# Academich/translation-transformer

Measured on AMD Instinct MI355X. Metric: reactions/sec (SMILES decoded), greedy speculative, higher is better.
Workload: dtype f32

## Files before the change

include/ttx.h:

```cpp
#ifndef TTX_H
#define TTX_H

#include <stdint.h>

#ifdef __cplusplus
extern "C" {
#endif

#define TTX_ABI_VERSION 4

typedef enum ttx_status {
  TTX_OK = 0,
  TTX_ERR_INVALID = -1,
  TTX_ERR_HIP = -2,
  TTX_ERR_NO_DEVICE = -3,
  TTX_ERR_REFERENCE = -4,
  TTX_ERR_NOMEM = -5,
  TTX_ERR_ROW_REPLAY = -6,
  TTX_ERR_MAX_STEPS = -7
} ttx_status;

typedef struct ttx_config {
  int32_t vocab_size;
  int32_t src_vocab_size;
// ... 230 lines not shown
                           float* d_kcache, float* d_vcache, int64_t cache_layer_stride, int64_t cache_seq_stride, int N, int D, int d,
                           int B, int Ld, const int32_t* d_pos2, const float* d_qkv_probe, int64_t probe_layer_stride, void* stream);

int ttx_debug_probe_split(ttx_session* s, const int32_t* d_act_idx, const int32_t* d_pred_probe, const int32_t* d_drafts, int B, int N,
                          int D, int n_active, int32_t* d_act2, int32_t* d_pos2, int32_t* result, void* stream);

int ttx_debug_merge_pred(ttx_session* s, const int32_t* d_pos2, const int32_t* d_pred_probe, const int32_t* d_pred2, int32_t* d_pred,
                         int B, int N, int D, int n_active, void* stream);

int ttx_debug_probe_split_select(ttx_session* s, const int32_t* d_act_idx, const int32_t* d_pred_probe, const int32_t* d_drafts, int B,
                                 int N, int D, int n_active, int32_t* d_act2, int32_t* d_pos2, int32_t* d_draft_mask, int32_t* d_row_base,
                                 int32_t* d_row_map, int32_t* result, void* stream);
int ttx_debug_merge_pred_select(ttx_session* s, const int32_t* d_pos2, const int32_t* d_pred_probe, const int32_t* d_pred2,
                                int32_t* d_pred, int B, int N, int D, int n_active, const int32_t* d_row_base,
                                const int32_t* d_draft_mask, void* stream);
int ttx_debug_kvcopy_select(ttx_session* s, const int32_t* d_rec, int n_copy, const float* d_qkv, int64_t qkv_layer_stride,
                            float* d_kcache, float* d_vcache, int64_t cache_layer_stride, int64_t cache_seq_stride, int N, int D, int d,
                            int B, int Ld, const int32_t* d_pos2, const float* d_qkv_probe, int64_t probe_layer_stride,
                            const int32_t* d_row_base, const int32_t* d_draft_mask, void* stream);
int ttx_debug_embed_select(ttx_session* s, const float* d_table, int V, const float* d_pe, int pe_rows, int d, float* d_x,
                           const int32_t* d_act_idx, const int32_t* d_front, const int32_t* d_gen, int gen_ld, const int32_t* d_drafts,
                           int B, int N, int D, int n_active, const int32_t* d_row_map, int m_rows, void* stream);
int ttx_debug_attn_select(ttx_session* s, const float* d_q, int ldq, const float* d_k, const float* d_v, int ldkv, float* d_out, int H,
                          float scale, int Lk, const int32_t* d_tok, int pad, const uint8_t* d_key_pad, const int32_t* d_act_idx,
                          const int32_t* d_front, const int32_t* d_src_of, const int32_t* d_src_len, const float* d_kcache,
                          const float* d_vcache, int64_t cache_seq_stride, const int32_t* d_cache_slot, int gen_ld, int N, int D, int mode,
                          int groups, int n_active, int max_keys, int kernel, int32_t* kernel_id, const int32_t* d_row_base,
                          const int32_t* d_draft_mask, void* stream);

int ttx_pool_last_counters(ttx_session* s, int64_t* counters);

int ttx_attn_staged_key_limit(int head_dim, int q_per_group);

#ifdef __cplusplus
}
#endif
#endif
```

translation-transformer_amd/_native.py:

```python
from __future__ import annotations

import ctypes as C
import os
import subprocess
from pathlib import Path

PKG_DIR = Path(__file__).resolve().parent
CSRC = PKG_DIR / "csrc"
INCLUDE = PKG_DIR.parent / "include"
LIB_PATH = PKG_DIR / "libttx_hip.so"
UNITS = [CSRC / "ttx_api.hip", CSRC / "ttx_gemm.hip", CSRC / "ttx_attn.hip"]
HEADERS = [CSRC / "ttx_internal.h", CSRC / "ttx_common.hip.h", CSRC / "ttx_loop_kernels.hip.h", CSRC / "ttx_metrics.hip.h",
           CSRC / "ttx_score.hip.h", CSRC / "ttx_select.h", CSRC / "ttx_tokenizer.h", INCLUDE / "ttx.h"]
SOURCES = UNITS + HEADERS
OBJ_DIR = CSRC / "build"

TTX_OK, TTX_ERR_INVALID, TTX_ERR_HIP, TTX_ERR_NO_DEVICE, TTX_ERR_REFERENCE, TTX_ERR_NOMEM = 0, -1, -2, -3, -4, -5
TTX_ERR_ROW_REPLAY = -6
TTX_ERR_MAX_STEPS = -7
TTX_ACT_NONE, TTX_ACT_RELU, TTX_ACT_GELU = 0, 1, 2
ACTIVATIONS = {"relu": TTX_ACT_RELU, "gelu": TTX_ACT_GELU}


def activation_code(activation: str) -> int:
# ... 117 lines not shown
    "ttx_tokenizer_encode": (C.c_int, [_VP, C.c_char_p, _VP, _I]),
    "ttx_tokenizer_encode_batch": (C.c_int, [_VP, C.POINTER(C.c_char_p), _I, _VP, _I]),
    "ttx_tokenizer_decode": (C.c_int, [_VP, _VP, _I, _VP, _I]),
    "ttx_debug_step_snapshot": (C.c_int, [_VP, C.POINTER(C.c_int32), _VP, _VP, _VP, _VP]),
    "ttx_debug_gemm_bench": (C.c_int, [_VP, _I, _I, _I, _I, _I, _I, C.POINTER(C.c_double), C.POINTER(C.c_double)]),
    "ttx_debug_gemm": (C.c_int, [_VP, _VP, _I, _VP, _I, _VP, _VP, _I, _VP, _I, _I, _I, _I, _I, C.c_int64, _I, _I,
                                 C.POINTER(C.c_int32), _VP]),
    "ttx_debug_gemm_act": (C.c_int, [_VP, _VP, _I, _VP, _I, _VP, _VP, _I, _VP, _I, _I, _I, _I, _I, C.c_int64, _I, _I,
                                     C.POINTER(C.c_int32), _VP]),
    "ttx_debug_finish_ln": (C.c_int, [_VP, _VP, _I, C.c_int64, _VP, _VP, _VP, _VP, _VP, _VP, _VP, _VP, _VP, _I, _I, C.c_float, _VP]),
    "ttx_debug_attn": (C.c_int, [_VP, _VP, _I, _VP, _VP, _I, _VP, _I, C.c_float, _I, _I, _VP, _I, _VP, _VP, _VP, _VP, _VP, _VP, _VP, _VP,
                                 C.c_int64, _VP, _I, _I, _I, _I, _I, _I, _I, _I, C.POINTER(C.c_int32), _VP]),
    "ttx_debug_attn_hd": (C.c_int, [_VP, _VP, _I, _VP, _VP, _I, _VP, _I, _I, C.c_float, _I, _I, _VP, _I, _VP, _VP, _VP, _VP, _VP, _VP, _VP,
                                    _VP, C.c_int64, _VP, _I, _I, _I, _I, _I, _I, _I, _I, C.POINTER(C.c_int32), _VP]),
    "ttx_debug_attn_as": (C.c_int, [_VP, _VP, _I, _VP, _VP, _I, _VP, _I, _I, C.c_float, _I, _I, _VP, _I, _VP, _VP, _VP, _VP, _VP, _VP, _VP,
                                    _VP, C.c_int64, _VP, _I, _I, _I, _I, _I, _I, _I, _I, C.POINTER(C.c_int32), _I, _I, _VP]),
    "ttx_debug_argmax": (C.c_int, [_VP, _VP, _I, _VP, _VP, _I, _VP]),
    "ttx_debug_embed": (C.c_int, [_VP, _VP, _I, _VP, _I, _I, _VP, _VP, _I, _I, _VP, _VP, _VP, _I, _VP, _I, _I, _I, _I, _I, _VP]),
    "ttx_debug_accept": (C.c_int, [_VP, C.POINTER(DebugAcceptArgs), C.POINTER(C.c_int64), _VP]),
    "ttx_debug_kvcopy": (C.c_int, [_VP, _VP, _I, _VP, C.c_int64, _VP, _VP, C.c_int64, C.c_int64, _I, _I, _I, _I, _I, _VP]),
    "ttx_debug_kvcopy_split": (C.c_int, [_VP, _VP, _I, _VP, C.c_int64, _VP, _VP, C.c_int64, C.c_int64, _I, _I, _I, _I, _I, _VP, _VP,
                                         C.c_int64, _VP]),
    "ttx_debug_probe_split": (C.c_int, [_VP, _VP, _VP, _VP, _I, _I, _I, _I, _VP, _VP, C.POINTER(C.c_int32), _VP]),
    "ttx_debug_merge_pred": (C.c_int, [_VP, _VP, _VP, _VP, _VP, _I, _I, _I, _I, _VP]),
    "ttx_debug_probe_split_select": (C.c_int, [_VP, _VP, _VP, _VP, _I, _I, _I, _I, _VP, _VP, _VP, _VP, _VP, C.POINTER(C.c_int32), _VP]),
    "ttx_debug_merge_pred_select": (C.c_int, [_VP, _VP, _VP, _VP, _VP, _I, _I, _I, _I, _VP, _VP, _VP]),
    "ttx_debug_kvcopy_select": (C.c_int, [_VP, _VP, _I, _VP, C.c_int64, _VP, _VP, C.c_int64, C.c_int64, _I, _I, _I, _I, _I, _VP, _VP,
                                          C.c_int64, _VP, _VP, _VP]),
    "ttx_debug_embed_select": (C.c_int, [_VP, _VP, _I, _VP, _I, _I, _VP, _VP, _VP, _VP, _I, _VP, _I, _I, _I, _I, _VP, _I, _VP]),
    "ttx_debug_attn_select": (C.c_int, [_VP, _VP, _I, _VP, _VP, _I, _VP, _I, C.c_float, _I, _VP, _I, _VP, _VP, _VP, _VP, _VP, _VP, _VP,
                                        C.c_int64, _VP, _I, _I, _I, _I, _I, _I, _I, _I, C.POINTER(C.c_int32), _VP, _VP, _VP]),
    "ttx_pool_last_counters": (C.c_int, [_VP, C.POINTER(C.c_int64)]),
    "ttx_attn_staged_key_limit": (C.c_int, [_I, _I]),
    "ttx_last_kernel_profile": (C.c_int, [_VP, C.POINTER(C.c_double), C.POINTER(C.c_int64), C.POINTER(C.c_double)]),
}

_lib = None


def hipcc_path() -> str:
    for cand in (os.environ.get("HIPCC"), "/opt/rocm/bin/hipcc", "hipcc"):
        if cand and (os.path.isabs(cand) and os.path.exists(cand) or not os.path.isabs(cand)):
            return cand
    return "hipcc"


def needs_build() -> bool:
    if not LIB_PATH.exists():
        return True
    t = LIB_PATH.stat().st_mtime
    return any(src.stat().st_mtime > t for src in SOURCES)


def build(force: bool = False, verbose: bool = False) -> Path:
    if not force and not needs_build():
        return LIB_PATH
    OBJ_DIR.mkdir(exist_ok=True)
    flags = ["--offload-arch=gfx950", "-O3", "-std=c++17", "-fPIC", f"-I{INCLUDE}"] + os.environ.get("TTX_HIPCC_FLAGS", "").split()
    newest_header = max(h.stat().st_mtime for h in HEADERS)
    jobs, objs = [], []
    for unit in UNITS:
        obj = OBJ_DIR / (unit.stem + ".o")
        objs.append(str(obj))
        if not force and obj.exists() and obj.stat().st_mtime > max(unit.stat().st_mtime, newest_header) \
                and not os.environ.get("TTX_HIPCC_FLAGS"):
            continue
# ... 41 lines not shown
```

translation-transformer_amd/csrc/ttx_api.hip:

```cpp
#include "ttx_internal.h"
#include "ttx_loop_kernels.hip.h"
#include "ttx_metrics.hip.h"
#include "ttx_score.hip.h"
#include "ttx_tokenizer.h"

#include <algorithm>
#include <chrono>
#include <cmath>
#include <cstdio>
#include <cstdlib>
#include <cstring>
#include <mutex>
#include <type_traits>

using namespace ttx;

static thread_local std::string g_err;

int ttx::fail(int code, const std::string& msg) {
  g_err = msg;
  return code;
}

static void layout_add(ttx_model* m, const std::string& name, size_t numel, size_t* off_out) {
// ... 249 lines not shown
    if (hipMemset(b.p, 0xFF, want) != hipSuccess) return fail(TTX_ERR_HIP, "hipMemset (poison) failed");
    (void)hipDeviceSynchronize();
  }
  return TTX_OK;
}

extern "C" int ttx_session_create(ttx_model* m, ttx_session** out) {
  if (!m || !out) return fail(TTX_ERR_INVALID, "null argument");
  HIP_TRY(hipSetDevice(m->device));
  ttx_session* s = new ttx_session();
  s->m = m;
  if (hipHostMalloc((void**)&s->host_info, sizeof(HostInfo), hipHostMallocMapped) != hipSuccess ||
      hipHostMalloc((void**)&s->probe_info, sizeof(ProbeInfo), hipHostMallocMapped) != hipSuccess ||
      hipHostMalloc((void**)&s->host_state, sizeof(DecState), hipHostMallocDefault) != hipSuccess) {
    if (s->host_info) (void)hipHostFree(s->host_info);
    if (s->probe_info) (void)hipHostFree(s->probe_info);
    if (s->host_state) (void)hipHostFree(s->host_state);
    delete s;
    return fail(TTX_ERR_NOMEM, "hipHostMalloc failed");
  }
  std::memset(s->host_info, 0, sizeof(HostInfo));
  std::memset(s->probe_info, 0, sizeof(ProbeInfo));
  HIP_TRY(hipEventCreate(&s->ev_a));
  HIP_TRY(hipEventCreate(&s->ev_b));
  HIP_TRY(hipEventCreate(&s->ev_c));
  HIP_TRY(hipEventCreateWithFlags(&s->ev_done, hipEventDisableTiming));
  s->use_graphs = getenv("TTX_NO_GRAPH") == nullptr;
  const char* pf = getenv("TTX_PROFILE_GEMM");
  s->profile = pf && pf[0] == '1';
  if (const char* e = getenv("TTX_SMALL_ROWS")) s->small_rows = std::max(0, atoi(e));
  if (const char* e = getenv("TTX_FFN2_SLAB_ROWS")) s->ffn2_slab_rows = std::max(0, atoi(e));
  if (const char* e = getenv("TTX_QKV_SMALL_ROWS")) s->qkv_small_rows = std::max(0, atoi(e));
  if (const char* e = getenv("TTX_ATTN_FALLBACK")) s->attn_fallback = atoi(e) != 0;
  s->host_timing = getenv("TTX_HOST_TIMING") != nullptr;
  m->n_sessions++;
  *out = s;
  return TTX_OK;
}

extern "C" void ttx_session_destroy(ttx_session* s) {
  if (!s) return;
  if (s->host_timing && s->host_launches)
    fprintf(stderr, "[ttx host timing] hipGraphLaunch: %lld launches, %.1f us each\n", s->host_launches,
            s->host_launch_us / (double)s->host_launches);
  if (s->host_timing && s->host_captures)
    fprintf(stderr, "[ttx host timing] graphs captured: %lld, %.1f us each\n", s->host_captures,
            s->host_capture_us / (double)s->host_captures);
  if (s->dead) {
    delete s;
    return;
  }
  release_retired();
  (void)hipDeviceSynchronize();
  for (Buf* b : s->all)
    if (b->p) (void)hipFree(b->p);
  if (s->host_info) (void)hipHostFree(s->host_info);
  if (s->probe_info) (void)hipHostFree(s->probe_info);
  if (s->beam_host) (void)hipHostFree(s->beam_host);
  if (s->bp_host) (void)hipHostFree(s->bp_host);
  s->drop_graphs();
  release_own_stream(s);
  if (s->ev_done) (void)hipEventDestroy(s->ev_done);
  if (s->host_state) (void)hipHostFree(s->host_state);
  for (auto& e : s->ev_pool) { (void)hipEventDestroy(e.first); (void)hipEventDestroy(e.second); }
  if (s->ev_a) (void)hipEventDestroy(s->ev_a);
  if (s->ev_b) (void)hipEventDestroy(s->ev_b);
// ... 2782 lines not shown
  MergePredArgs mp{};
  mp.st = dst; mp.pos2 = d_pos2; mp.pred_probe = d_pred_probe; mp.pred2 = d_pred2; mp.pred = d_pred; mp.RPS = step_rps(N, D);
  mp.row_base = d_row_base; mp.draft_mask = d_draft_mask; mp.D = D;
  hipLaunchKernelGGL(k_merge_pred, dim3(cdiv(B * mp.RPS, 256)), dim3(256), 0, st, mp);
  hipError_t err = hipGetLastError();
  const hipError_t esync = hipStreamSynchronize(st);
  (void)hipFree(dst);
  HIP_TRY(err);
  HIP_TRY(esync);
  return TTX_OK;
}

extern "C" int ttx_debug_merge_pred(ttx_session* s, const int32_t* d_pos2, const int32_t* d_pred_probe, const int32_t* d_pred2,
                                    int32_t* d_pred, int B, int N, int D, int n_active, void* stream) {
  return merge_pred_debug(s, d_pos2, d_pred_probe, d_pred2, d_pred, B, N, D, n_active, nullptr, nullptr, stream);
}

extern "C" int ttx_debug_merge_pred_select(ttx_session* s, const int32_t* d_pos2, const int32_t* d_pred_probe, const int32_t* d_pred2,
                                           int32_t* d_pred, int B, int N, int D, int n_active, const int32_t* d_row_base,
                                           const int32_t* d_draft_mask, void* stream) {
  if ((d_row_base != nullptr) != (d_draft_mask != nullptr))
    return fail(TTX_ERR_INVALID, "ttx_debug_merge_pred_select: row_base and draft_mask come together");
  return merge_pred_debug(s, d_pos2, d_pred_probe, d_pred2, d_pred, B, N, D, n_active, d_row_base, d_draft_mask, stream);
}

extern "C" int ttx_pool_last_counters(ttx_session* s, int64_t* counters) {
  if (!s || !counters) return fail(TTX_ERR_INVALID, "null argument to ttx_pool_last_counters");
  for (int i = 0; i < 7; ++i) counters[i] = s->pool_counters[i];
  return TTX_OK;
}

extern "C" int ttx_attn_staged_key_limit(int head_dim, int q_per_group) { return attn_staged_key_limit(head_dim, q_per_group); }

extern "C" int ttx_last_kernel_profile(ttx_session* s, double* gemm_ms, int64_t* gemm_launches, double* empty_pair_ms) {
  if (!s) return fail(TTX_ERR_INVALID, "null session");
  if (gemm_ms) *gemm_ms = s->prof_ms;
  if (gemm_launches) *gemm_launches = s->prof_launches;
  s->prof_ms = 0;
  s->prof_launches = 0;
  if (empty_pair_ms) *empty_pair_ms = s->prof_empty_pair_ms < 0 ? 0.0 : s->prof_empty_pair_ms;
  return TTX_OK;
}
```

translation-transformer_amd/csrc/ttx_attn.hip:

```cpp
#include "ttx_internal.h"

#include <algorithm>

namespace ttx {

constexpr int ATT_MAXQ = 16;
constexpr int ATT_SQ = ATT_MAXQ + 1;

__host__ __device__ inline size_t attn_lds_bytes(int max_keys, int dh) {
  return sizeof(float) * ((size_t)ATT_MAXQ * dh + (size_t)max_keys * ATT_SQ + ATT_MAXQ);
}

template <int DH, class KeyPtr, class Vis>
__device__ __forceinline__ void attn_core(const float* __restrict__ q, int ldq, int nq, int nk, KeyPtr keyptr, Vis vis,
                                          float* __restrict__ out, int ldo, float scale, float* lds) {
  const int lane = threadIdx.x & 63;
  float* Qs = lds;
  float* S = lds + ATT_MAXQ * DH;
  float* inv = S + (size_t)nk * ATT_SQ;

  for (int e = lane * 4; e < nq * DH; e += 256) {
    const int i = e / DH, c = e % DH;
    *reinterpret_cast<float4*>(&Qs[i * DH + c]) = *reinterpret_cast<const float4*>(q + (size_t)i * ldq + c);
  }
// ... 824 lines not shown
    float mx, rs, fa, fb;
    f32x16 oi;
    a3_tile_partial<MODE>(a, cu, cur, cq, it * 32, r, h, magic, mx, rs, oi);
    a3_fold(m, l, mx, rs, fa, fb);
#pragma unroll
    for (int i = 0; i < 16; ++i) o[i] = __fmaf_rn(o[i], fa, __fmul_rn(oi[i], fb));
    cur = nxt;
    if (!last) {
      ++it;
      continue;
    }
    if (SEL ? cq.orow >= 0 : r < cu.nq) {
      const float inv = l > 0.f ? 1.0f / l : 0.f;
      float* op = cu.out + (size_t)(SEL ? cq.orow : r) * a.d + 4 * h;
#pragma unroll
      for (int v = 0; v < 4; ++v) {
        f32x4 w = {o[4 * v] * inv, o[4 * v + 1] * inv, o[4 * v + 2] * inv, o[4 * v + 3] * inv};
        *reinterpret_cast<f32x4*>(op + 8 * v) = w;
      }
    }
    if (!more) break;
    cu = nu;
    cq = nq;
    un += W;
    nu = unit(min(un, n_units - 1));
    it = 0;
    m = -INFINITY;
    l = 0.f;
#pragma unroll
    for (int i = 0; i < 16; ++i) o[i] = 0.f;
  }
}

static constexpr size_t kAttn2LdsLimit = 150 * 1024;

template <int MODE, int DH>
static int launch_attn_mode(ttx_session* s, hipStream_t st, const AttnArgs& a, int groups, int H, int q_per_group, int max_keys, int N, int D1) {
  if (groups <= 0 || q_per_group <= 0) return TTX_OK;
  constexpr bool step = (MODE == ATT_STEP_SELF || MODE == ATT_STEP_CROSS);
  const int D = D1 - 1;
  const int force = s->attn_force;
  const bool want3 = force ? (force == AK_ATTN3 || force == AK_ATTN3S) : !s->attn_fallback;
  const bool want2 = force ? force == AK_ATTN2 : !s->attn_fallback;
  if ((force == AK_ATTN3 || force == AK_ATTN3S) && !(step && H % 4 == 0 && DH == ATT_DH))
    return fail(TTX_ERR_INVALID, "k_attn3 / k_attn3s serve the step modes at head dimension 32 with a head count that is a multiple of 4");
  const bool sel = a.row_base != nullptr;
  if (sel && !(step && DH == ATT_DH && H % 4 == 0 && want3 && a.draft_mask && N <= 32 && D >= 1))
    return fail(TTX_ERR_INVALID, "draft select runs on k_attn3 / k_attn3s only: a step launch at head dimension 32, a head count that is a "
                                 "multiple of 4, 1 <= N <= 32 and D >= 1");
  if constexpr (step && DH == ATT_DH) {
    if (H % 4 == 0 && want3) {
      const int qtiles = cdiv(q_per_group, A3_QT);
      const int keys3 = (MODE == ATT_STEP_SELF) ? max_keys + 1 + N * std::max(D, 0) : max_keys;
      const size_t lds3 = sizeof(float) * (size_t)A3_PART * cdiv(keys3, 32);
      bool split = s->attn_split != 0 && (s->attn_split > 0 || (long long)groups * H * qtiles < TTX_A3_SPLIT_BELOW) && lds3 <= 64 * 1024;
      if (force == AK_ATTN3 && lds3 > 64 * 1024) return fail(TTX_ERR_INVALID, "k_attn3: the parked tile partials exceed 64 KB of LDS");
      if (force) split = (force == AK_ATTN3);
      s->last_attn_kernel = split ? AK_ATTN3 : AK_ATTN3S;
      if (split) {
        if (sel) hipLaunchKernelGGL((k_attn3<MODE, true>), dim3(groups, H, qtiles), dim3(256), lds3, st, a);
        else hipLaunchKernelGGL((k_attn3<MODE, false>), dim3(groups, H, qtiles), dim3(256), lds3, st, a);
      } else {
        const long long units = (long long)groups * H * qtiles;
        const int wgs = (int)std::min<long long>((units + 3) / 4, (long long)TTX_A3S_WGS_PER_CU * s->m->n_cu);
        if (sel) hipLaunchKernelGGL((k_attn3s<MODE, true>), dim3(wgs), dim3(256), 0, st, a, H, qtiles);
        else hipLaunchKernelGGL((k_attn3s<MODE, false>), dim3(wgs), dim3(256), 0, st, a, H, qtiles);
      }
      HIP_TRY(hipGetLastError());
      return TTX_OK;
    }
  }
  const int draft_keys = (D > 0) ? (std::min(N, (A2_QT + D - 2) / D + 1)) * D : 0;
  const int keys2 = (MODE == ATT_STEP_SELF) ? max_keys + 1 + draft_keys : max_keys;
  const size_t lds2 = attn2_lds_bytes(keys2, a2_qcap(q_per_group), DH);
  if (force == AK_ATTN2 && !(lds2 <= kAttn2LdsLimit && attn2_fits(keys2, DH)))
    return fail(TTX_ERR_INVALID, "k_attn2: more keys than its register and LDS images hold");
  bool fits2 = lds2 <= kAttn2LdsLimit && attn2_fits(keys2, DH);
  if (step && s->attn_sel_N > 0) {
    const int cN = s->attn_sel_N, cD = s->attn_sel_D;
    const int c_draft = (cD > 0) ? (std::min(cN, (A2_QT + cD - 2) / cD + 1)) * cD : 0;
    const int c_keys2 = (MODE == ATT_STEP_SELF) ? max_keys + 1 + c_draft : max_keys;
    fits2 = fits2 && attn2_lds_bytes(c_keys2, a2_qcap(step_rps(cN, cD)), DH) <= kAttn2LdsLimit && attn2_fits(c_keys2, DH);
  }
  if (fits2 && want2) {
    s->last_attn_kernel = AK_ATTN2;
    const int tiles = cdiv(q_per_group, A2_QT);
    bool& attr_set = s->attr_attn2[DH == ATT_DH ? 0 : 1][MODE];
    if (lds2 > 64 * 1024 && !attr_set) {
      HIP_TRY(hipFuncSetAttribute(reinterpret_cast<const void*>(&k_attn2<MODE, DH>), hipFuncAttributeMaxDynamicSharedMemorySize,
                                  (int)kAttn2LdsLimit));
      attr_set = true;
    }
    hipLaunchKernelGGL((k_attn2<MODE, DH>), dim3(groups, H, tiles), dim3(256), lds2, st, a);
    HIP_TRY(hipGetLastError());
    return TTX_OK;
  }
  const int keys1 = (MODE == ATT_STEP_SELF) ? max_keys + q_per_group : max_keys;
  const size_t lds = attn_lds_bytes(keys1, DH);
  if (lds > kAttn2LdsLimit) return fail(TTX_ERR_INVALID, "sequence too long for the attention kernels' LDS score buffer");
  if (lds > 64 * 1024)
    HIP_TRY(hipFuncSetAttribute(reinterpret_cast<const void*>(&k_attn<MODE, DH>), hipFuncAttributeMaxDynamicSharedMemorySize, (int)lds));
  s->last_attn_kernel = AK_ATTN;
  hipLaunchKernelGGL((k_attn<MODE, DH>), dim3(groups, H, cdiv(q_per_group, ATT_MAXQ)), dim3(64), lds, st, a);
  HIP_TRY(hipGetLastError());
  return TTX_OK;
}

template <int DH>
static int launch_attn_dh(int mode, ttx_session* s, hipStream_t st, const AttnArgs& a, int groups, int H, int q_per_group, int max_keys,
                          int N, int D1) {
  switch (mode) {
    case ATT_ENC: return launch_attn_mode<ATT_ENC, DH>(s, st, a, groups, H, q_per_group, max_keys, N, D1);
    case ATT_FULL_SELF: return launch_attn_mode<ATT_FULL_SELF, DH>(s, st, a, groups, H, q_per_group, max_keys, N, D1);
    case ATT_FULL_CROSS: return launch_attn_mode<ATT_FULL_CROSS, DH>(s, st, a, groups, H, q_per_group, max_keys, N, D1);
    case ATT_STEP_SELF: return launch_attn_mode<ATT_STEP_SELF, DH>(s, st, a, groups, H, q_per_group, max_keys, N, D1);
    case ATT_STEP_CROSS: return launch_attn_mode<ATT_STEP_CROSS, DH>(s, st, a, groups, H, q_per_group, max_keys, N, D1);
  }
  return fail(TTX_ERR_INVALID, "unknown attention mode");
}

int launch_attn(int mode, ttx_session* s, hipStream_t st, const AttnArgs& a, int groups, int H, int q_per_group, int max_keys,
                int N, int D1) {
  if (H > 0 && a.d == H * 32) return launch_attn_dh<32>(mode, s, st, a, groups, H, q_per_group, max_keys, N, D1);
  if (H > 0 && a.d == H * 64) return launch_attn_dh<64>(mode, s, st, a, groups, H, q_per_group, max_keys, N, D1);
  return fail(TTX_ERR_INVALID, "attention kernels exist for head dimensions 32 and 64");
}

int attn_staged_key_limit(int head_dim, int q_per_group) {
  if ((head_dim != 32 && head_dim != 64) || q_per_group <= 0) return 0;
  int keys = 32 * a2_vsteps(head_dim);
  while (keys > 0 && attn2_lds_bytes(keys, a2_qcap(q_per_group), head_dim) > kAttn2LdsLimit) keys -= 32;
  return keys;
}

static bool attn_aligned16(const void* p) { return (reinterpret_cast<uintptr_t>(p) & 15) == 0; }

int attn_debug(ttx_session* s, const AttnArgs& in, int H, int head_dim, int mode, int groups, int n_active, int max_keys, int kernel,
               int32_t* kernel_id, hipStream_t st) {
  if (!s) return fail(TTX_ERR_INVALID, "null session");
  if (head_dim != 32 && head_dim != 64) return fail(TTX_ERR_INVALID, "ttx_debug_attn_hd: head_dim is 32 or 64");
  if (mode < ATT_ENC || mode > ATT_STEP_CROSS || kernel < 0 || kernel > AK_ATTN3S)
    return fail(TTX_ERR_INVALID, "ttx_debug_attn: mode is 0..4, kernel 0..4");
  if (H <= 0 || groups <= 0 || max_keys <= 0) return fail(TTX_ERR_INVALID, "ttx_debug_attn: H, groups and max_keys must be positive");
  const bool step = (mode == ATT_STEP_SELF || mode == ATT_STEP_CROSS);
  const bool cross = (mode == ATT_FULL_CROSS || mode == ATT_STEP_CROSS);
  AttnArgs a = in;
  a.d = H * head_dim;
  if (!a.q || !a.k || !a.v || !a.out) return fail(TTX_ERR_INVALID, "ttx_debug_attn: q, k, v and out are required");
  if (cross ? !a.key_pad : !a.tok) return fail(TTX_ERR_INVALID, "ttx_debug_attn: self modes need tok, cross modes key_pad");
  if (step && !a.act_idx) return fail(TTX_ERR_INVALID, "ttx_debug_attn: the step modes need act_idx");
  if (mode == ATT_STEP_SELF && (!a.front || !a.kcache || !a.vcache))
    return fail(TTX_ERR_INVALID, "ttx_debug_attn: STEP_SELF needs front, kcache and vcache");
  if ((a.ldq & 3) || (a.ldkv & 3) || a.ldq < a.d || a.ldkv < a.d)
    return fail(TTX_ERR_INVALID, "ttx_debug_attn: ldq and ldkv must be multiples of 4 that cover d = head_dim * H");
  for (const void* p : {(const void*)a.q, (const void*)a.k, (const void*)a.v, (const void*)a.out, (const void*)a.kcache, (const void*)a.vcache})
    if (!attn_aligned16(p)) return fail(TTX_ERR_INVALID, "ttx_debug_attn: float operands must be 16-byte aligned");
  int q_per_group = a.L;
  if (step) {
    if (a.N < 1 || a.D < 0) return fail(TTX_ERR_INVALID, "ttx_debug_attn: step modes need N >= 1 and D >= 0");
    if (n_active < 0 || n_active > groups) return fail(TTX_ERR_INVALID, "ttx_debug_attn: n_active must lie in [0, groups]");
    if (mode == ATT_STEP_SELF && (a.gen_ld <= 0 || a.cache_seq_stride <= 0 || (a.cache_seq_stride & 3)))
      return fail(TTX_ERR_INVALID, "ttx_debug_attn: STEP_SELF needs gen_ld > 0 and a cache_seq_stride that is a positive multiple of 4");
    q_per_group = step_rps(a.N, a.D);
  } else if (a.L <= 0 || (mode != ATT_FULL_CROSS && max_keys < a.L)) {
    return fail(TTX_ERR_INVALID, "ttx_debug_attn: L must be positive and max_keys cover it");
  }
  if (cross && (a.Lk <= 0 || max_keys < a.Lk)) return fail(TTX_ERR_INVALID, "ttx_debug_attn: Lk must be positive and max_keys cover it");
  HIP_TRY(hipSetDevice(s->m->device));
  DecState* dst = nullptr;
  if (step) {
    HIP_TRY(hipMalloc((void**)&dst, sizeof(DecState)));
    hipError_t e = hipMemsetAsync(dst, 0, sizeof(DecState), st);
    if (e == hipSuccess) e = hipMemsetD32Async(reinterpret_cast<hipDeviceptr_t>(&dst->n_active), n_active, 1, st);
    if (e != hipSuccess) { (void)hipFree(dst); HIP_TRY(e); }
    a.st = dst;
// ... 17 lines not shown
```

translation-transformer_amd/csrc/ttx_internal.h:

```cpp
#pragma once
#include "ttx.h"
#include "ttx_common.hip.h"

#include <map>
#include <set>
#include <string>
#include <utility>
#include <vector>

namespace ttx {
struct BeamHost;
struct BeamPoolHost;
}

struct LayerW {
  size_t sa_in_w, sa_in_b, sa_out_w, sa_out_b;
  size_t ca_in_w, ca_in_b, ca_out_w, ca_out_b;
  size_t l1_w, l1_b, l2_w, l2_b;
  size_t n1_w, n1_b, n2_w, n2_b, n3_w, n3_b;
};

struct ttx_model {
  ttx_config cfg;
  int device;
  int activation = TTX_ACT_RELU;
  int n_sessions = 0;

  int n_cu = 256;
  float* blob = nullptr;
  size_t blob_floats = 0;
  std::map<std::string, std::pair<size_t, size_t>> index;
  std::vector<LayerW> enc, dec;
  size_t src_emb, tgt_emb, enc_norm_w, enc_norm_b, dec_norm_w, dec_norm_b, cls_w, cls_b, pe;
  size_t cross_kv_w, cross_kv_b;
  const float* p(size_t off) const { return blob + off; }
};

struct Buf {
  void* p = nullptr;
  size_t cap = 0;
  uint64_t* owner_gen = nullptr;
  template <typename T> T* as() const { return reinterpret_cast<T*>(p); }
};

enum GemmVariant { GV_BIG = 0, GV_SMALL = 1, GV_BIG_FFN2_SLABS = 2, GV_MID = 3 };

enum GemmKernelId { GK_GEMM3 = 1, GK_GEMM_TN = 2, GK_GEMM24_4 = 3, GK_GEMM24_0 = 4, GK_GEMM2_1 = 5, GK_GEMM2_2 = 6, GK_GEMM2_4 = 7,
                    GK_GEMM2_0 = 8, GK_BODY_128x64 = 16 };

enum AttnKernelId { AK_ATTN = 1, AK_ATTN2 = 2, AK_ATTN3 = 3, AK_ATTN3S = 4 };

enum GraphSite { GS_STEP_SPECULATIVE = 0, GS_STEP_GREEDY = 1, GS_STEP_ROW_RULE = 2, GS_STEP_POOL = 3, GS_BEAM_ITER = 4, GS_BEAM_POOL_ITER = 5 };
typedef std::vector<int> GraphKey;

struct GraphCache {
  std::map<GraphKey, hipGraphExec_t> map;
  std::set<GraphKey> warmed;
  size_t limit;
  explicit GraphCache(size_t limit_) : limit(limit_) {}
  void clear() {
    for (auto& kv : map) (void)hipGraphExecDestroy(kv.second);
    map.clear(); warmed.clear();
  }
};

#define TTX_SESSION_BUFS(X)                                                                                                      \
                                                                      \
  X(x) X(x1) X(x2) X(xf) X(ao) X(q2) X(hbuf) X(slab) X(qkv) X(logits) X(ckv)                                                      \
                                                                                                                    \
  X(tok_src) X(src_valid) X(memory) X(memkv)                                                                                     \
                                                                                                               \
  X(tok_tgt) X(mem_pad_tmp)                                                                                                      \
   \
  X(ev_logits) X(ev_pred) X(ev_nll)                                                                                              \
   \
                                                                                                      \
  X(sc_src_of)                                                                                                                   \
                                                                                                                       \
  X(drafts) X(gen) X(front) X(act_idx) X(rec) X(pred) X(state) X(kcache) X(vcache) X(src32) X(outbuf) X(haspad) X(traj)           \
  X(fin_step)                                                                                                                    \
                                                                                            \
  X(rstep) X(row_of) X(src_len) X(new_slot) X(pool_io) X(memkv_new) X(valid_new) X(drafts_new)                                    \
       \
// ... 17 lines not shown
#ifndef TTX_BIG_MIN_TILES
#define TTX_BIG_MIN_TILES 400
#endif
struct ttx_session {
  ttx_model* m;
  std::vector<Buf*> all;
  TTX_SESSION_BUFS(TTX_DECLARE_BUF)
  Buf tk[2], tv[2];
  int snap_B = 0, snap_rps = 0, snap_gen_ld = 0, snap_step = 0;
  ttx::ProbeInfo* probe_info = nullptr;
  long long pool_counters[7] = {};
  ttx::BeamHost* beam_host = nullptr;
  ttx::BeamPoolHost* bp_host = nullptr;
  ttx::HostInfo* host_info = nullptr;
  hipStream_t own_stream = nullptr;
  uint64_t alloc_generation = 0;
  uint64_t graphs_generation = 0;
  bool dead = false;
  bool use_graphs = true;
  GraphCache step_graphs{512};
  GraphCache iter_graphs{256};
  hipEvent_t ev_done = nullptr;
  void drop_graphs() { step_graphs.clear(); iter_graphs.clear(); }
  void graphs_current() { if (graphs_generation != alloc_generation) { drop_graphs(); graphs_generation = alloc_generation; } }
  ttx::DecState* host_state = nullptr;
  bool attr_attn2[2][8] = {};
  bool attr_select = false, attr_step = false, attr_topk = false, attr_pool_select = false;
  int qkv_small_rows = 800;
  int small_rows = 2000;
  int ffn2_slab_rows = 5600;
  int big_min_tiles = TTX_BIG_MIN_TILES;
  int last_gemm_kernel = 0, last_gemm_big_min_tiles = 0;
  int attn_split = -1;
  bool attn_fallback = false;
  int attn_force = 0;
  int attn_sel_N = 0, attn_sel_D = 0;
  int last_attn_kernel = 0;
  bool profile = false;
  std::vector<std::pair<hipEvent_t, hipEvent_t>> ev_pool;
  size_t ev_used = 0;
  double prof_ms = 0;
  double prof_empty_pair_ms = -1;
  long long prof_launches = 0;
  bool host_timing = false;
  double host_launch_us = 0;
  long long host_captures = 0;
  double host_capture_us = 0;
  long long host_launches = 0;
  hipEvent_t ev_a = nullptr, ev_b = nullptr, ev_c = nullptr;
  ttx_session() {
    TTX_SESSION_BUFS(TTX_REGISTER_BUF)
    for (Buf* b : {&tk[0], &tk[1], &tv[0], &tv[1]}) all.push_back(b);
    for (Buf* b : all) b->owner_gen = &alloc_generation;
  }
};

namespace ttx {

int fail(int code, const std::string& msg);

#define HIP_TRY(expr)                                                                                  \
  do {                                                                                                 \
    hipError_t _e = (expr);                                                                            \
    if (_e != hipSuccess)                                                                              \
      return ttx::fail(TTX_ERR_HIP, std::string(#expr) + ": " + hipGetErrorString(_e) + " (" __FILE__ ":" + \
                                        std::to_string(__LINE__) + ")");                               \
  } while (0)

#define TTX_TRY(expr)        \
  do {                       \
// ... 33 lines not shown
```

translation-transformer_amd/model.py:

```python
from __future__ import annotations

import ctypes as C
import os
import math
from typing import NamedTuple

import numpy as np
import torch

from . import _native as N


def reference_pe_table(emb: int, max_len: int = 5000) -> torch.Tensor:
    pe = torch.zeros(max_len, emb)
    position = torch.arange(0, max_len, dtype=torch.float).unsqueeze(1)
    div_term = torch.exp(torch.arange(0, emb, 2).float() * (-math.log(10000.0) / emb))
    pe[:, 0::2] = torch.sin(position * div_term)
    pe[:, 1::2] = torch.cos(position * div_term)
    return torch.vstack((torch.zeros(1, emb), pe)).contiguous()


def _strip(state: dict) -> dict:
    if any(k.startswith("model.") for k in state):
        return {k[len("model."):]: v for k, v in state.items() if k.startswith("model.")}
# ... 258 lines not shown
                            row_base: torch.Tensor | None, draft_mask: torch.Tensor | None) -> None:
        assert kcache.stride() == vcache.stride()
        N.check(self._lib.ttx_debug_kvcopy_select(self._session, rec.data_ptr(), int(n_copy), qkv.data_ptr(), int(qkv.stride(0)),
                                                  kcache.data_ptr(), vcache.data_ptr(), int(kcache.stride(0)), int(kcache.stride(1)),
                                                  int(n), int(d), int(width), int(B), int(qkv.shape[0]), self._ptr(pos2),
                                                  self._ptr(qkv_probe), 0 if qkv_probe is None else int(qkv_probe.stride(0)),
                                                  self._ptr(row_base), self._ptr(draft_mask), self._stream()))

    def debug_embed_select(self, table: torch.Tensor, pe: torch.Tensor, x: torch.Tensor, act_idx: torch.Tensor, front: torch.Tensor,
                           gen: torch.Tensor, drafts: torch.Tensor, B: int, n: int, d: int, n_active: int,
                           row_map: torch.Tensor | None, m_rows: int) -> None:
        N.check(self._lib.ttx_debug_embed_select(self._session, table.data_ptr(), int(table.shape[0]), pe.data_ptr(), int(pe.shape[0]),
                                                 int(table.shape[1]), x.data_ptr(), act_idx.data_ptr(), front.data_ptr(),
                                                 gen.data_ptr(), int(gen.stride(0)), drafts.data_ptr(), int(B), int(n), int(d),
                                                 int(n_active), self._ptr(row_map), int(m_rows), self._stream()))

    def debug_attn_select(self, mode: int, q: torch.Tensor, k: torch.Tensor, v: torch.Tensor, out: torch.Tensor, heads: int,
                          scale: float, groups: int, max_keys: int, row_base: torch.Tensor | None, draft_mask: torch.Tensor | None,
                          Lk: int = 0, tok: torch.Tensor | None = None, pad: int = 0, key_pad: torch.Tensor | None = None,
                          act_idx: torch.Tensor | None = None, front: torch.Tensor | None = None, src_of: torch.Tensor | None = None,
                          src_len: torch.Tensor | None = None, kcache: torch.Tensor | None = None, vcache: torch.Tensor | None = None,
                          cache_seq_stride: int = 0, cache_slot: torch.Tensor | None = None, gen_ld: int = 0, n: int = 1, d: int = 0,
                          n_active: int = 0, kernel: int = 0, **unused) -> int:
        kid = C.c_int32(0)
        assert k.stride(0) == v.stride(0)
        N.check(self._lib.ttx_debug_attn_select(self._session, q.data_ptr(), q.stride(0), k.data_ptr(), v.data_ptr(), k.stride(0),
                                                out.data_ptr(), int(heads), float(scale), int(Lk), self._ptr(tok), int(pad),
                                                self._ptr(key_pad), self._ptr(act_idx), self._ptr(front), self._ptr(src_of),
                                                self._ptr(src_len), self._ptr(kcache), self._ptr(vcache), int(cache_seq_stride),
                                                self._ptr(cache_slot), int(gen_ld), int(n), int(d), int(mode), int(groups),
                                                int(n_active), int(max_keys), int(kernel), C.byref(kid), self._ptr(row_base),
                                                self._ptr(draft_mask), self._stream()))
        return int(kid.value)

    POOL_COUNTERS = ("steps", "split_steps", "slot_steps_probed", "slots_matched", "drafts_matched", "rows_executed", "draft_select")

    def pool_last_counters(self, session=None) -> dict:
        words = (C.c_int64 * 7)()
        N.check(self._lib.ttx_pool_last_counters(self._session if session is None else session, words))
        return dict(zip(self.POOL_COUNTERS, (int(v) for v in words)))

    @staticmethod
    def attn_staged_key_limit(head_dim: int, q_per_group: int) -> int:
        return int(N.lib().ttx_attn_staged_key_limit(int(head_dim), int(q_per_group)))

    def close(self) -> None:
        if getattr(self, "_score_session", None):
            self._lib.ttx_session_destroy(self._score_session)
            self._score_session = None
        for extra in getattr(self, "_pool", [])[1:]:
            self._lib.ttx_session_destroy(extra)
        self._pool = None
        if getattr(self, "_session", None):
            self._lib.ttx_session_destroy(self._session)
            self._session = None
        if getattr(self, "_model", None):
            self._lib.ttx_model_destroy(self._model)
            self._model = None

    def __del__(self):
        try:
            self.close()
        except Exception:
            pass

    def _tokens(self, t: torch.Tensor) -> torch.Tensor:
# ... 181 lines not shown
```

Baseline: 21430.

## Add single-row step attention kernel with two heads per 64-thread block

Adds k_attn1, a step-attention kernel for one query row at head dimension 32. Each 64-lane block handles two heads, keeps K tiles staged in LDS and prefetches the next tile while an online softmax accumulates. By default it replaces k_attn3s for unsplit, non-select launches with one query per group, aiming to cut launch width and LDS overhead for tiny decode steps. It also adds a per-session bitmask of attention kernels used, plus a debug accessor. The risk is lower occupancy and serial key tiles on long keys, and speculative launches may not reach this path at all.

```diff
diff --git a/include/ttx.h b/include/ttx.h
--- a/include/ttx.h
+++ b/include/ttx.h
@@ -286,6 +286,8 @@
 
 int ttx_attn_staged_key_limit(int head_dim, int q_per_group);
 
+int ttx_debug_attn_kernels_seen(ttx_session* s);
+
 #ifdef __cplusplus
 }
 #endif
diff --git a/translation-transformer_amd/_native.py b/translation-transformer_amd/_native.py
--- a/translation-transformer_amd/_native.py
+++ b/translation-transformer_amd/_native.py
@@ -173,6 +173,7 @@
                                         C.c_int64, _VP, _I, _I, _I, _I, _I, _I, _I, _I, C.POINTER(C.c_int32), _VP, _VP, _VP]),
     "ttx_pool_last_counters": (C.c_int, [_VP, C.POINTER(C.c_int64)]),
     "ttx_attn_staged_key_limit": (C.c_int, [_I, _I]),
+    "ttx_debug_attn_kernels_seen": (C.c_int, [_VP]),
     "ttx_last_kernel_profile": (C.c_int, [_VP, C.POINTER(C.c_double), C.POINTER(C.c_int64), C.POINTER(C.c_double)]),
 }
 
diff --git a/translation-transformer_amd/csrc/ttx_api.hip b/translation-transformer_amd/csrc/ttx_api.hip
--- a/translation-transformer_amd/csrc/ttx_api.hip
+++ b/translation-transformer_amd/csrc/ttx_api.hip
@@ -305,6 +305,7 @@
   if (const char* e = getenv("TTX_FFN2_SLAB_ROWS")) s->ffn2_slab_rows = std::max(0, atoi(e));
   if (const char* e = getenv("TTX_QKV_SMALL_ROWS")) s->qkv_small_rows = std::max(0, atoi(e));
   if (const char* e = getenv("TTX_ATTN_FALLBACK")) s->attn_fallback = atoi(e) != 0;
+  if (const char* e = getenv("TTX_ATTN_ROW")) s->attn_row = atoi(e) != 0 ? 1 : 0;
   s->host_timing = getenv("TTX_HOST_TIMING") != nullptr;
   m->n_sessions++;
   *out = s;
@@ -3153,6 +3154,11 @@
 
 extern "C" int ttx_attn_staged_key_limit(int head_dim, int q_per_group) { return attn_staged_key_limit(head_dim, q_per_group); }
 
+extern "C" int ttx_debug_attn_kernels_seen(ttx_session* s) {
+  if (!s) return fail(TTX_ERR_INVALID, "null session");
+  return (int)s->attn_kernels_seen;
+}
+
 extern "C" int ttx_last_kernel_profile(ttx_session* s, double* gemm_ms, int64_t* gemm_launches, double* empty_pair_ms) {
   if (!s) return fail(TTX_ERR_INVALID, "null session");
   if (gemm_ms) *gemm_ms = s->prof_ms;
diff --git a/translation-transformer_amd/csrc/ttx_attn.hip b/translation-transformer_amd/csrc/ttx_attn.hip
--- a/translation-transformer_amd/csrc/ttx_attn.hip
+++ b/translation-transformer_amd/csrc/ttx_attn.hip
@@ -880,6 +880,98 @@
   }
 }
 
+template <int MODE>
+__global__ __launch_bounds__(64) void k_attn1(AttnArgs a) {
+  static_assert(MODE == ATT_STEP_SELF || MODE == ATT_STEP_CROSS, "k_attn1 serves the verify step");
+  typedef float f32x4 __attribute__((ext_vector_type(4)));
+  __shared__ __attribute__((aligned(16))) float a1_p[2][64];
+  constexpr int A1_KROW = 36;
+  __shared__ __attribute__((aligned(16))) float a1_k[64 * A1_KROW + 32];
+  const int slot = blockIdx.x;
+  if (slot >= a.st->n_active) return;
+  const int lane = threadIdx.x, r = lane & 31, ho = (lane >> 5) * ATT_DH;
+  const A3Unit c = a3_unit<MODE, false>(a, slot, 2 * (int)blockIdx.y, 0, 1, 0u);
+  float q[32];
+#pragma unroll
+  for (int g = 0; g < 8; ++g) {
+    const f32x4 v = *reinterpret_cast<const f32x4*>(c.q + ho + 4 * g);
+    q[4 * g] = __fmul_rn(v.x, a.scale); q[4 * g + 1] = __fmul_rn(v.y, a.scale);
+    q[4 * g + 2] = __fmul_rn(v.z, a.scale); q[4 * g + 3] = __fmul_rn(v.w, a.scale);
+  }
+  auto a1_row = [&](int key, const float* lin, const float* stp) -> const float* {
+    if constexpr (MODE == ATT_STEP_SELF) return key < c.f ? lin + key * a.d : stp;
+    else return lin + key * a.ldkv;
+  };
+  const int kc4 = (lane & 15) * 4, ksub = lane >> 4;
+  float* const kst = a1_k + (lane & 8) * (A1_KROW * 4 + 4) + (lane & 7) * 4;
+  const float* const krd = a1_k + (lane >> 5) * (A1_KROW * 32 + 32) + r * A1_KROW;
+  f32x4 kg[8];
+  int own;
+  auto load_k = [&](int key0) {
+#pragma unroll
+    for (int j = 0; j < 8; ++j)
+      kg[j] = *reinterpret_cast<const f32x4*>(a1_row(min(key0 + 4 * j + ksub, c.nk - 1), c.klin, c.kb) + kc4);
+    own = a3_keyown<MODE>(a, c, min(key0 + r, c.nk - 1));
+  };
+  float m = -INFINITY, l = 0.f, o = 0.f;
+  if (c.ntiles > 0) load_k(0);
+  for (int it = 0; it < c.ntiles; ++it) {
+    const int key0 = it * 32;
+    float vv[32];
+#pragma unroll
+    for (int j = 0; j < 32; ++j) {
+      vv[j] = a1_row(min(key0 + j, c.nk - 1), c.vlin, c.vb)[ho + r];
+    }
+    asm volatile("" ::: "memory");
+#pragma unroll
+    for (int j = 0; j < 8; ++j) *reinterpret_cast<f32x4*>(kst + (4 * j + ksub) * A1_KROW) = kg[j];
+    __syncthreads();
+    f32x4 kk[8];
+#pragma unroll
+    for (int g = 0; g < 8; ++g) kk[g] = *reinterpret_cast<const f32x4*>(krd + 4 * g);
+    float s = 0.f;
+#pragma unroll
+    for (int g = 0; g < 4; ++g)
+#pragma unroll
+      for (int e = 0; e < 4; ++e) {
+        s = __fmaf_rn(kk[2 * g][e], q[8 * g + e], s);
+        s = __fmaf_rn(kk[2 * g + 1][e], q[8 * g + 4 + e], s);
+      }
+    s = (key0 + r < c.nk && own != 0) ? s : -INFINITY;
+    asm volatile("" ::: "memory");
+    __syncthreads();
+    load_k(min(it + 1, c.ntiles - 1) * 32);
+    asm volatile("" ::: "memory");
+    float mx = s;
+#pragma unroll
+    for (int off = 16; off >= 1; off >>= 1) mx = fmaxf(mx, __shfl_xor(mx, off));
+    const float base = (mx == -INFINITY) ? 0.f : mx;
+    float* pl = a1_p[it & 1];
+    pl[lane] = __expf(s - base);
+    __syncthreads();
+    float p[32];
+#pragma unroll
+    for (int g = 0; g < 8; ++g) {
+      const f32x4 v = *reinterpret_cast<const f32x4*>(pl + ho + 4 * g);
+      p[4 * g] = v.x; p[4 * g + 1] = v.y; p[4 * g + 2] = v.z; p[4 * g + 3] = v.w;
+    }
+    float rs0 = 0.f, rs1 = 0.f, oi = 0.f;
+#pragma unroll
+    for (int t = 0; t < 16; ++t) {
+      const int j = (t & 3) + 8 * (t >> 2);
+      rs0 = __fadd_rn(rs0, p[j]);
+      rs1 = __fadd_rn(rs1, p[j + 4]);
+      oi = __fmaf_rn(vv[j], p[j], oi);
+      oi = __fmaf_rn(vv[j + 4], p[j + 4], oi);
+    }
+    float fa, fb;
+    a3_fold(m, l, mx, __fadd_rn(rs0, rs1), fa, fb);
+    o = __fmaf_rn(o, fa, __fmul_rn(oi, fb));
+  }
+  const float inv = l > 0.f ? 1.0f / l : 0.f;
+  c.out[ho + r] = o * inv;
+}
+
 static constexpr size_t kAttn2LdsLimit = 150 * 1024;
 
 template <int MODE, int DH>
@@ -888,8 +980,10 @@
   constexpr bool step = (MODE == ATT_STEP_SELF || MODE == ATT_STEP_CROSS);
   const int D = D1 - 1;
   const int force = s->attn_force;
-  const bool want3 = force ? (force == AK_ATTN3 || force == AK_ATTN3S) : !s->attn_fallback;
+  const bool want3 = force ? (force == AK_ATTN3 || force == AK_ATTN3S || force == AK_ATTN1) : !s->attn_fallback;
   const bool want2 = force ? force == AK_ATTN2 : !s->attn_fallback;
+  if (force == AK_ATTN1 && !(step && H % 4 == 0 && DH == ATT_DH && q_per_group == 1))
+    return fail(TTX_ERR_INVALID, "k_attn1 serves one-row step launches (N * D = 0) at head dimension 32 with a head count that is a multiple of 4");
   if ((force == AK_ATTN3 || force == AK_ATTN3S) && !(step && H % 4 == 0 && DH == ATT_DH))
     return fail(TTX_ERR_INVALID, "k_attn3 / k_attn3s serve the step modes at head dimension 32 with a head count that is a multiple of 4");
   const bool sel = a.row_base != nullptr;
@@ -904,8 +998,11 @@
       bool split = s->attn_split != 0 && (s->attn_split > 0 || (long long)groups * H * qtiles < TTX_A3_SPLIT_BELOW) && lds3 <= 64 * 1024;
       if (force == AK_ATTN3 && lds3 > 64 * 1024) return fail(TTX_ERR_INVALID, "k_attn3: the parked tile partials exceed 64 KB of LDS");
       if (force) split = (force == AK_ATTN3);
-      s->last_attn_kernel = split ? AK_ATTN3 : AK_ATTN3S;
-      if (split) {
+      const bool row = force ? force == AK_ATTN1 : (q_per_group == 1 && !sel && s->attn_row != 0 && (s->attn_row > 0 || !split));
+      s->last_attn_kernel = row ? AK_ATTN1 : split ? AK_ATTN3 : AK_ATTN3S;
+      if (row) {
+        hipLaunchKernelGGL((k_attn1<MODE>), dim3(groups, H / 2), dim3(64), 0, st, a);
+      } else if (split) {
         if (sel) hipLaunchKernelGGL((k_attn3<MODE, true>), dim3(groups, H, qtiles), dim3(256), lds3, st, a);
         else hipLaunchKernelGGL((k_attn3<MODE, false>), dim3(groups, H, qtiles), dim3(256), lds3, st, a);
       } else {
@@ -969,9 +1066,12 @@
 
 int launch_attn(int mode, ttx_session* s, hipStream_t st, const AttnArgs& a, int groups, int H, int q_per_group, int max_keys,
                 int N, int D1) {
-  if (H > 0 && a.d == H * 32) return launch_attn_dh<32>(mode, s, st, a, groups, H, q_per_group, max_keys, N, D1);
-  if (H > 0 && a.d == H * 64) return launch_attn_dh<64>(mode, s, st, a, groups, H, q_per_group, max_keys, N, D1);
-  return fail(TTX_ERR_INVALID, "attention kernels exist for head dimensions 32 and 64");
+  if (!(H > 0 && (a.d == H * 32 || a.d == H * 64))) return fail(TTX_ERR_INVALID, "attention kernels exist for head dimensions 32 and 64");
+  s->last_attn_kernel = 0;
+  const int rc = a.d == H * 32 ? launch_attn_dh<32>(mode, s, st, a, groups, H, q_per_group, max_keys, N, D1)
+                               : launch_attn_dh<64>(mode, s, st, a, groups, H, q_per_group, max_keys, N, D1);
+  if (rc == TTX_OK && s->last_attn_kernel) s->attn_kernels_seen |= 1u << s->last_attn_kernel;
+  return rc;
 }
 
 int attn_staged_key_limit(int head_dim, int q_per_group) {
@@ -987,8 +1087,8 @@
                int32_t* kernel_id, hipStream_t st) {
   if (!s) return fail(TTX_ERR_INVALID, "null session");
   if (head_dim != 32 && head_dim != 64) return fail(TTX_ERR_INVALID, "ttx_debug_attn_hd: head_dim is 32 or 64");
-  if (mode < ATT_ENC || mode > ATT_STEP_CROSS || kernel < 0 || kernel > AK_ATTN3S)
-    return fail(TTX_ERR_INVALID, "ttx_debug_attn: mode is 0..4, kernel 0..4");
+  if (mode < ATT_ENC || mode > ATT_STEP_CROSS || kernel < 0 || kernel > AK_ATTN1)
+    return fail(TTX_ERR_INVALID, "ttx_debug_attn: mode is 0..4, kernel 0..5");
   if (H <= 0 || groups <= 0 || max_keys <= 0) return fail(TTX_ERR_INVALID, "ttx_debug_attn: H, groups and max_keys must be positive");
   const bool step = (mode == ATT_STEP_SELF || mode == ATT_STEP_CROSS);
   const bool cross = (mode == ATT_FULL_CROSS || mode == ATT_STEP_CROSS);
diff --git a/translation-transformer_amd/csrc/ttx_internal.h b/translation-transformer_amd/csrc/ttx_internal.h
--- a/translation-transformer_amd/csrc/ttx_internal.h
+++ b/translation-transformer_amd/csrc/ttx_internal.h
@@ -48,7 +48,7 @@
 enum GemmKernelId { GK_GEMM3 = 1, GK_GEMM_TN = 2, GK_GEMM24_4 = 3, GK_GEMM24_0 = 4, GK_GEMM2_1 = 5, GK_GEMM2_2 = 6, GK_GEMM2_4 = 7,
                     GK_GEMM2_0 = 8, GK_BODY_128x64 = 16 };
 
-enum AttnKernelId { AK_ATTN = 1, AK_ATTN2 = 2, AK_ATTN3 = 3, AK_ATTN3S = 4 };
+enum AttnKernelId { AK_ATTN = 1, AK_ATTN2 = 2, AK_ATTN3 = 3, AK_ATTN3S = 4, AK_ATTN1 = 5 };
 
 enum GraphSite { GS_STEP_SPECULATIVE = 0, GS_STEP_GREEDY = 1, GS_STEP_ROW_RULE = 2, GS_STEP_POOL = 3, GS_BEAM_ITER = 4, GS_BEAM_POOL_ITER = 5 };
 typedef std::vector<int> GraphKey;
@@ -132,10 +132,12 @@
   int big_min_tiles = TTX_BIG_MIN_TILES;
   int last_gemm_kernel = 0, last_gemm_big_min_tiles = 0;
   int attn_split = -1;
+  int attn_row = -1;
   bool attn_fallback = false;
   int attn_force = 0;
   int attn_sel_N = 0, attn_sel_D = 0;
   int last_attn_kernel = 0;
+  unsigned attn_kernels_seen = 0;
   bool profile = false;
   std::vector<std::pair<hipEvent_t, hipEvent_t>> ev_pool;
   size_t ev_used = 0;
diff --git a/translation-transformer_amd/model.py b/translation-transformer_amd/model.py
--- a/translation-transformer_amd/model.py
+++ b/translation-transformer_amd/model.py
@@ -314,6 +314,12 @@
                                                 int(n_active), int(max_keys), int(kernel), C.byref(kid), self._ptr(row_base),
                                                 self._ptr(draft_mask), self._stream()))
         return int(kid.value)
+
+    def attn_kernels_seen(self, session=None) -> set:
+        mask = int(self._lib.ttx_debug_attn_kernels_seen(self._session if session is None else session))
+        if mask < 0:
+            N.check(mask)
+        return {k for k in range(1, 32) if mask >> k & 1}
 
     POOL_COUNTERS = ("steps", "split_steps", "slot_steps_probed", "slots_matched", "drafts_matched", "rows_executed", "draft_select")
 
```

Measured after the change: 22980, median of 6. +7.2%, better.
